# lattice/quda

Hardware: AMD Instinct MI355X
Metric: wilson_clover_cg_gflops (higher is better)
Workload: dtype double-half; 1 GPU; model=wilson_clover_eo_pc_cg, lattice_per_gpu=32x32x32x64, global_batch=1, seq_len=2097152, parallelism=dd_t1, gauge_recon_sloppy=12

## Files before the change

### csrc/bindings.cpp

```cpp
#include <torch/extension.h>
#include <c10/hip/HIPStream.h>
#include <hip/hip_runtime.h>

#include "launchers.h"

namespace {

int prec_of(const at::Tensor &t) {
  switch (t.scalar_type()) {
    case at::kDouble: return 0;
    case at::kFloat: return 1;
    case at::kHalf: return 2;
    case at::kFloat8_e4m3fn: return 3;
    default: TORCH_CHECK(false, "unsupported dtype");
  }
}

void *ptr_or_null(const at::Tensor &t) {
  return t.numel() ? t.data_ptr() : nullptr;
}

BlasField field_of(const at::Tensor &data, const at::Tensor &norm, long Vcb) {
  return BlasField{ptr_or_null(data), ptr_or_null(norm), Vcb};
}
// ... 263 lines not shown
}

static at::Tensor blas_op(int64_t op, double a, double b, at::Tensor x,
                          at::Tensor x_n, at::Tensor y, at::Tensor y_n,
                          int64_t Vcb, int64_t sites, double c2 = 0.0,
                          double d2 = 0.0, int64_t ncomp = 24,
                          bool deterministic = false,
                          c10::optional<at::Tensor> z = c10::nullopt,
                          c10::optional<at::Tensor> z_n = c10::nullopt,
                          c10::optional<at::Tensor> w = c10::nullopt,
                          c10::optional<at::Tensor> w_n = c10::nullopt) {
  TORCH_CHECK(op != BLAS_TRIPLE_CG_DEV,
              "blas_op: BLAS_TRIPLE_CG_DEV takes a device accumulator — call "
              "triple_cg_dev");
  BlasCall c{};
  c.op = (int)op;
  c.prec = prec_of(x);
  c.a = a;
  c.b = b;
  c.c = c2;
  c.d = d2;
  c.ncomp = (int)ncomp;
  c.det = deterministic;
  c.x = field_of(x, x_n, Vcb);
  c.y = field_of(y, y_n, Vcb);
  if (z) c.z = field_of(*z, *z_n, Vcb);
  if (w) c.w = field_of(*w, *w_n, Vcb);
  c.sites = sites;
  at::Tensor result;
  bool reduction = (op == BLAS_AXPY_NORM2 || op == BLAS_XMY_NORM2 ||
                    op == BLAS_NORM2 || op == BLAS_REDOT || op == BLAS_CDOT ||
                    op == BLAS_TRIPLE_CG);
  if (reduction) {
    if (deterministic) {
      long g = (sites + 255) / 256;
      if (g > 2048) g = 2048;
      result = at::zeros({g, 2}, x.options().dtype(at::kDouble));
    } else {
      result = at::zeros({2}, x.options().dtype(at::kDouble));
    }
    c.result = result.data_ptr<double>();
  }
  launch_blas(c, stream());
  check_launch("blas_op");
  if (reduction && deterministic) result = result.sum(0);
  return result;
}

static void triple_cg_dev(double r2_old, at::Tensor acc, at::Tensor clear,
                          at::Tensor p, at::Tensor p_n, at::Tensor Ap,
                          at::Tensor Ap_n, at::Tensor x, at::Tensor x_n,
                          at::Tensor r, at::Tensor r_n, int64_t Vcb,
                          int64_t sites, int64_t ncomp, at::Tensor slots,
                          int64_t nslots, int64_t slot_stride) {
  auto ok = [&](const at::Tensor &t) {
    return t.scalar_type() == at::kDouble && t.is_contiguous() &&
           t.device() == p.device();
  };
  TORCH_CHECK(ok(acc) && acc.numel() >= 2,
              "triple_cg_dev: acc must hold 2 float64 on the fields' device");
  TORCH_CHECK(clear.numel() == 0 || ok(clear),
              "triple_cg_dev: clear must be empty or float64 on the device");
  if (clear.numel()) {
    auto lo = (const char *)clear.data_ptr(), hi = lo + clear.numel() * 8;
    auto a0 = (const char *)acc.data_ptr();
    TORCH_CHECK(a0 + 16 <= lo || a0 >= hi,
                "triple_cg_dev: clear must not overlap acc");
  }
  TORCH_CHECK(nslots == 0 ||
              (ok(slots) && nslots >= 1 && nslots <= 64 && slot_stride >= 1 &&
               slots.numel() >= (nslots - 1) * slot_stride + 1),
              "triple_cg_dev: slots must hold nslots <= 64 strided float64");
  BlasCall c{};
  c.op = BLAS_TRIPLE_CG_DEV;
  c.prec = prec_of(p);
  c.a = r2_old;
  c.ncomp = (int)ncomp;
  c.x = field_of(p, p_n, Vcb);
  c.y = field_of(Ap, Ap_n, Vcb);
  c.z = field_of(x, x_n, Vcb);
  c.w = field_of(r, r_n, Vcb);
  c.sites = sites;
  c.result = acc.data_ptr<double>();
  c.clear = clear.numel() ? clear.data_ptr<double>() : nullptr;
  c.clear_n = clear.numel();
  c.nslots = (int)nslots;
  c.slot_stride = (int)slot_stride;
  c.slots = nslots ? slots.data_ptr<double>() : nullptr;
  launch_blas(c, stream());
  check_launch("triple_cg_dev");
}

static void convert(at::Tensor dst, at::Tensor dst_n, at::Tensor src,
                    at::Tensor src_n, int64_t Vcb, int64_t sites,
                    int64_t ncomp = 24) {
  launch_convert(field_of(dst, dst_n, Vcb), prec_of(dst),
                 field_of(src, src_n, Vcb), prec_of(src), sites, (int)ncomp,
                 stream());
  check_launch("convert");
}

static void clover_apply(at::Tensor out, at::Tensor out_n, at::Tensor in,
                         at::Tensor in_n, at::Tensor clover, int64_t parity,
                         int64_t Vcb, int64_t v_stride, int64_t s_offset) {
  CloverApplyCall c{};
  c.out = field_of_off(out, out_n, v_stride ? v_stride : Vcb, s_offset);
  c.in = field_of_off(in, in_n, v_stride ? v_stride : Vcb, s_offset);
  c.clover = clover.data_ptr();
  c.parity = (int)parity;
  c.Vcb = Vcb;
  c.sites = Vcb;
  c.prec = prec_of(out);
  launch_clover_apply(c, stream());
  check_launch("clover_apply");
}

static void twist_apply(at::Tensor out, at::Tensor out_n, at::Tensor in,
                        at::Tensor in_n, double b_re, double b_im,
                        int64_t Vcb, int64_t sites, int64_t tau3_vcb = 0,
                        bool acc = false) {
  TwistApplyCall c{};
  c.out = field_of(out, out_n, Vcb);
  c.in = field_of(in, in_n, Vcb);
  c.b_re = b_re;
  c.b_im = b_im;
  c.sites = sites;
  c.tau3_vcb = tau3_vcb;
  c.acc = acc;
  c.prec = prec_of(out);
  launch_twist_apply(c, stream());
  check_launch("twist_apply");
}

static void dwf5(at::Tensor out, at::Tensor out_n, at::Tensor in,
                 at::Tensor in_n, at::Tensor x, at::Tensor x_n,
                 int64_t Vcb4, int64_t Ls, bool xpay, bool dagger, double a,
                 double alpha, double beta, double mf, int64_t kind) {
  Dwf5Call c{};
  long stride = Vcb4 * Ls;
  c.out = field_of(out, out_n, stride);
  c.in = field_of(in, in_n, stride);
  c.x = field_of(x, x_n, stride);
  c.Vcb4 = Vcb4;
// ... 526 lines not shown
        py::arg("s_offsets") = std::vector<int64_t>{});
  m.def("flow_zmat_dir", &flow_zmat_dir, "wilson-flow Z = eps TA[S U^d]");
  m.def("flow_expmul_dir", &flow_expmul_dir, "U' = exp(Zc) U");
  m.def("stout_smear_dir", &stout_smear_dir,
        "native stout smear of one direction (exp via scale-and-square)");
  m.def("heatbath_sweep_dir", &heatbath_sweep_dir,
        "SU(2)-subgroup heatbath/overrelax update of one (parity, mu)");
  m.def("coarse_dslash_mfma", &coarse_dslash_mfma,
        "coarse-grid 9-matrix dslash on f32 MFMA tiles");
  m.def("dslash_staggered", &dslash_staggered, "naive staggered dslash");
  m.def("set_dslash_block", &set_dslash_block, "autotuner: dslash workgroup size");
  m.def("set_dslash_waves", &set_dslash_waves,
        "occupancy experiment: 0 default, 3 = 64-thread/3-wave variant "
        "(half/single/quarter; double keeps its default kernel)");
  m.def("set_dslash_lds", &set_dslash_lds,
        "LDS-tiled dslash policy: 1 = stage the in-spinor halo tile in LDS "
        "(half/quarter, local, tile-divisible dims)");
  m.def("get_dslash_block", &get_dslash_block, "current dslash workgroup size");
  m.def("get_dslash_lds", &get_dslash_lds, "current LDS-tiled dslash policy");
  m.def("get_dslash_waves", &get_dslash_waves, "current occupancy variant");
  m.def("ipc_get_handle", &ipc_get_handle, "hipIpcGetMemHandle of a tensor");
  m.def("ipc_open_handle", &ipc_open_handle, "open a peer IPC handle");
  m.def("ipc_close_handle", &ipc_close_handle, "close a peer IPC mapping");
  m.def("pack_face_ptr", &pack_face_ptr,
        "pack a halo face into a raw (IPC peer) pointer");
  m.def("dwf5", &dwf5, "DWF/Moebius 5th-dim ops (Ds apply / M5 inverse)");
  m.def("dwf_fused", &dwf_fused,
        "fused domain-wall kernel: out = [x +] a * W_chi (Dhat in), all Ls "
        "slices in one launch",
        py::arg("out"), py::arg("out_n"), py::arg("in"), py::arg("in_n"),
        py::arg("gauge"), py::arg("x"), py::arg("x_n"), py::arg("W"),
        py::arg("dims"), py::arg("parity_offset"), py::arg("Vcb"),
        py::arg("Ls"), py::arg("parity"), py::arg("dagger"), py::arg("xpay"),
        py::arg("a"), py::arg("recon"));
  m.def("set_dwf_fused_ns", &set_dwf_fused_ns,
        "fused domain-wall kernel: sites per workgroup for single/half "
        "(16 or 32)");
  m.attr("DWF_FUSED_LS_MAX") = (int)QA_DWF_FUSED_LS_MAX;
  m.def("zdwf5", &zdwf5, "zMobius per-slice-complex 5th-dim ops");
  m.def("eofa5", &eofa5, "EOFA rank-1 extended M5 ops");
  m.def("blas_op", &blas_op, "fused blas/reduction",
        py::arg("op"), py::arg("a"), py::arg("b"), py::arg("x"),
        py::arg("x_n"), py::arg("y"), py::arg("y_n"), py::arg("Vcb"),
        py::arg("sites"), py::arg("c2") = 0.0, py::arg("d2") = 0.0,
        py::arg("ncomp") = 24, py::arg("deterministic") = false,
        py::arg("z") = py::none(), py::arg("z_n") = py::none(),
        py::arg("w") = py::none(), py::arg("w_n") = py::none());
  m.def("triple_cg_dev", &triple_cg_dev,
        "fused CG update with alpha = r2_old / acc[0] formed on the device",
        py::arg("r2_old"), py::arg("acc"), py::arg("clear"), py::arg("p"),
        py::arg("p_n"), py::arg("Ap"), py::arg("Ap_n"), py::arg("x"),
        py::arg("x_n"), py::arg("r"), py::arg("r_n"), py::arg("Vcb"),
        py::arg("sites"), py::arg("ncomp"),
        py::arg("slots"), py::arg("nslots"), py::arg("slot_stride"));
  m.def("convert", &convert, "precision conversion copy", py::arg("dst"),
        py::arg("dst_n"), py::arg("src"), py::arg("src_n"), py::arg("Vcb"),
        py::arg("sites"), py::arg("ncomp") = 24);
  m.def("clover_apply", &clover_apply, "clover term apply",
        py::arg("out"), py::arg("out_n"), py::arg("in"), py::arg("in_n"),
        py::arg("clover"), py::arg("parity"), py::arg("Vcb"),
        py::arg("v_stride") = 0, py::arg("s_offset") = 0);
  m.def("twist_apply", &twist_apply, "twisted-mass T(b) apply",
        py::arg("out"), py::arg("out_n"), py::arg("in"), py::arg("in_n"),
        py::arg("b_re"), py::arg("b_im"), py::arg("Vcb"), py::arg("sites"),
        py::arg("tau3_vcb") = 0, py::arg("acc") = false);
  m.attr("BLAS_AXPY") = (int)BLAS_AXPY;
  m.attr("BLAS_AXPY_NORM2") = (int)BLAS_AXPY_NORM2;
  m.attr("BLAS_XPAY") = (int)BLAS_XPAY;
  m.attr("BLAS_AXPBY") = (int)BLAS_AXPBY;
  m.attr("BLAS_CAXPY") = (int)BLAS_CAXPY;
  m.attr("BLAS_XMY_NORM2") = (int)BLAS_XMY_NORM2;
  m.attr("BLAS_SCAL") = (int)BLAS_SCAL;
  m.attr("BLAS_NORM2") = (int)BLAS_NORM2;
  m.attr("BLAS_TRIPLE_CG") = (int)BLAS_TRIPLE_CG;
  m.attr("BLAS_TRIPLE_CG_DEV") = (int)BLAS_TRIPLE_CG_DEV;
  m.attr("BLAS_REDOT") = (int)BLAS_REDOT;
  m.attr("BLAS_CDOT") = (int)BLAS_CDOT;
  m.attr("BLAS_CAXPBY") = (int)BLAS_CAXPBY;
}
```

### csrc/blas.hip

```cpp
#include "common.h"
#include "reduce.h"

#define GRID_STRIDE(g, n)                                                     \
  for (long g = (long)blockIdx.x * blockDim.x + threadIdx.x; g < (n);         \
       g += (long)gridDim.x * blockDim.x)

template <typename A, bool NORM2>
__global__ __launch_bounds__(256) void k_axpy(
    typename A::R a, A x, A y, long sites, double *result, bool det) {
  using R = typename A::R;
  double acc = 0.0;
  GRID_STRIDE(g, sites) {
    cplx<R> xv[A::NCPLX], yv[A::NCPLX];
    x.load_v(xv, g);
    y.load_v(yv, g);
#pragma unroll
    for (int k = 0; k < A::NCPLX; ++k) {
      yv[k] = yv[k] + a * xv[k];
      if constexpr (NORM2)
        acc += (double)yv[k].re * yv[k].re + (double)yv[k].im * yv[k].im;
    }
    y.store_v(yv, g);
  }
  if constexpr (NORM2) block_atomic_add(acc, result, det, 2, 0);
// ... 114 lines not shown
  block_atomic_add(acc, result, det, 2, 0);
  if constexpr (KIND == 2) block_atomic_add(acc2, result, det, 2, 1);
}

template <typename AD, typename AS>
__global__ __launch_bounds__(256) void k_convert(AD dst, AS src, long sites) {
  using RS = typename AS::R;
  using RD = typename AD::R;
  static_assert(AD::NCPLX == AS::NCPLX);
  GRID_STRIDE(g, sites) {
    cplx<RS> v[AS::NCPLX];
    src.load_v(v, g);
    cplx<RD> o[AD::NCPLX];
#pragma unroll
    for (int k = 0; k < AS::NCPLX; ++k) o[k] = {(RD)v[k].re, (RD)v[k].im};
    dst.store_v(o, g);
  }
}

#include "launchers.h"

namespace {
constexpr int BLK = 256;
int grid_for(long sites) {
  long g = (sites + BLK - 1) / BLK;
  return (int)(g < 2048 ? g : 2048);
}
}

template <typename A>
__global__ __launch_bounds__(256) void k_triple_cg(
    typename A::R a, A p, A ap, A x, A r, long sites, double *result,
    bool det) {
  using R = typename A::R;
  double acc = 0.0;
  GRID_STRIDE(g, sites) {
    cplx<R> pv[A::NCPLX], av[A::NCPLX], xv[A::NCPLX], rv[A::NCPLX];
    p.load_v(pv, g);
    ap.load_v(av, g);
    x.load_v(xv, g);
    r.load_v(rv, g);
#pragma unroll
    for (int k = 0; k < A::NCPLX; ++k) {
      xv[k] = xv[k] + a * pv[k];
      rv[k] = rv[k] - a * av[k];
      acc += (double)rv[k].re * rv[k].re + (double)rv[k].im * rv[k].im;
    }
    x.store_v(xv, g);
    r.store_v(rv, g);
  }
  block_atomic_add(acc, result, det, 2, 0);
}

template <typename A>
__global__ __launch_bounds__(256) void k_triple_cg_dev(
    double r2_old, double *acc_out, double *clear, long clear_n,
    const double *slots, int nslots, int slot_stride, A p, A ap, A x, A r,
    long sites) {
  using R = typename A::R;
  if (clear && blockIdx.x == 0 && threadIdx.x < 64)
    for (long k = threadIdx.x; k < clear_n; k += 64) clear[k] = 0.0;
  double pAp;
  if (nslots > 0) {
    int lane = threadIdx.x & 63;
    double v = lane < nslots ? slots[(long)lane * slot_stride] : 0.0;
    v = wave_reduce(v);
    pAp = __shfl(v, 0, 64);
    if (blockIdx.x == 0 && threadIdx.x == 0) acc_out[0] = pAp;
  } else {
    pAp = acc_out[0];
  }
  if (pAp <= 0.0) return;
  const R a = (R)(r2_old / pAp);
  double acc = 0.0;
  GRID_STRIDE(g, sites) {
    cplx<R> pv[A::NCPLX], av[A::NCPLX], xv[A::NCPLX], rv[A::NCPLX];
    p.load_v(pv, g);
    ap.load_v(av, g);
    x.load_v(xv, g);
    r.load_v(rv, g);
#pragma unroll
    for (int k = 0; k < A::NCPLX; ++k) {
      xv[k] = xv[k] + a * pv[k];
      rv[k] = rv[k] - a * av[k];
      acc += (double)rv[k].re * rv[k].re + (double)rv[k].im * rv[k].im;
    }
    x.store_v(xv, g);
    r.store_v(rv, g);
  }
  block_atomic_add(acc, acc_out, false, 1, 1);
}

template <typename A>
static void blas_dispatch(const BlasCall &c, hipStream_t st) {
  using S = typename A::S;
  A x{(S *)c.x.data, (float *)c.x.norm, c.x.Vcb};
  A y{(S *)c.y.data, (float *)c.y.norm, c.y.Vcb};
  long n = c.sites;
  int gr = grid_for(n);
  using R = typename A::R;
  switch (c.op) {
    case BLAS_AXPY:
      hipLaunchKernelGGL((k_axpy<A, false>), dim3(gr), dim3(BLK), 0, st,
                         (R)c.a, x, y, n, nullptr, false);
      break;
    case BLAS_AXPY_NORM2:
      hipLaunchKernelGGL((k_axpy<A, true>), dim3(gr), dim3(BLK), 0, st,
                         (R)c.a, x, y, n, c.result, c.det);
      break;
    case BLAS_TRIPLE_CG: {
      A z{(S *)c.z.data, (float *)c.z.norm, c.z.Vcb};
      A w{(S *)c.w.data, (float *)c.w.norm, c.w.Vcb};
      hipLaunchKernelGGL((k_triple_cg<A>), dim3(gr), dim3(BLK), 0, st,
                         (R)c.a, x, y, z, w, n, c.result, c.det);
      break;
    }
    case BLAS_TRIPLE_CG_DEV: {
      A z{(S *)c.z.data, (float *)c.z.norm, c.z.Vcb};
      A w{(S *)c.w.data, (float *)c.w.norm, c.w.Vcb};
      hipLaunchKernelGGL((k_triple_cg_dev<A>), dim3(gr), dim3(BLK), 0, st,
                         c.a, c.result, c.clear, c.clear_n, c.slots, c.nslots,
                         c.slot_stride, x, y, z, w, n);
      break;
    }
    case BLAS_XPAY:
      hipLaunchKernelGGL((k_xpay<A>), dim3(gr), dim3(BLK), 0, st, x, (R)c.a, y, n);
      break;
    case BLAS_AXPBY:
      hipLaunchKernelGGL((k_axpby<A>), dim3(gr), dim3(BLK), 0, st, (R)c.a, x,
                         (R)c.b, y, n);
      break;
    case BLAS_CAXPY:
      hipLaunchKernelGGL((k_caxpy<A>), dim3(gr), dim3(BLK), 0, st, (R)c.a,
                         (R)c.b, x, y, n);
      break;
    case BLAS_CAXPBY:
      hipLaunchKernelGGL((k_caxpby<A>), dim3(gr), dim3(BLK), 0, st, (R)c.a,
                         (R)c.b, x, (R)c.c, (R)c.d, y, n);
      break;
    case BLAS_XMY_NORM2:
      hipLaunchKernelGGL((k_xmy_norm2<A>), dim3(gr), dim3(BLK), 0, st, x, y, n,
                         c.result, c.det);
      break;
    case BLAS_SCAL:
      hipLaunchKernelGGL((k_scal<A>), dim3(gr), dim3(BLK), 0, st, (R)c.a, x, n);
      break;
    case BLAS_NORM2:
      hipLaunchKernelGGL((k_reduce<A, 0>), dim3(gr), dim3(BLK), 0, st, x, y, n,
                         c.result, c.det);
      break;
    case BLAS_REDOT:
      hipLaunchKernelGGL((k_reduce<A, 1>), dim3(gr), dim3(BLK), 0, st, x, y, n,
                         c.result, c.det);
      break;
    case BLAS_CDOT:
      hipLaunchKernelGGL((k_reduce<A, 2>), dim3(gr), dim3(BLK), 0, st, x, y, n,
                         c.result, c.det);
      break;
  }
}

void launch_blas(const BlasCall &c, hipStream_t st) {
  if (c.ncomp == 6) {
    switch (c.prec) {
      case 0: blas_dispatch<StagAcc<PrecDouble>>(c, st); break;
      case 1: blas_dispatch<StagAcc<PrecSingle>>(c, st); break;
      case 2: blas_dispatch<StagAcc<PrecHalf>>(c, st); break;
      case 3: blas_dispatch<StagAcc<PrecQuarter>>(c, st); break;
    }
  } else {
    switch (c.prec) {
      case 0: blas_dispatch<SpinorAcc<PrecDouble>>(c, st); break;
      case 1: blas_dispatch<SpinorAcc<PrecSingle>>(c, st); break;
      case 2: blas_dispatch<SpinorAcc<PrecHalf>>(c, st); break;
      case 3: blas_dispatch<SpinorAcc<PrecQuarter>>(c, st); break;
    }
  }
}

template <template <typename> class AT, typename PD, typename PS>
static void conv(const BlasField &d, const BlasField &s, long sites, hipStream_t st) {
  auto da = AT<PD>{(typename PD::Store *)d.data, (float *)d.norm, d.Vcb};
  auto sa = AT<PS>{(typename PS::Store *)s.data, (float *)s.norm, s.Vcb};
  hipLaunchKernelGGL((k_convert<AT<PD>, AT<PS>>), dim3(grid_for(sites)),
                     dim3(BLK), 0, st, da, sa, sites);
}

template <template <typename> class AT>
static void conv_dispatch(const BlasField &dst, int pdst, const BlasField &src,
                          int psrc, long sites, hipStream_t st) {
  switch (pdst * 4 + psrc) {
    case 0 * 4 + 1: conv<AT, PrecDouble, PrecSingle>(dst, src, sites, st); break;
    case 0 * 4 + 2: conv<AT, PrecDouble, PrecHalf>(dst, src, sites, st); break;
    case 1 * 4 + 0: conv<AT, PrecSingle, PrecDouble>(dst, src, sites, st); break;
    case 1 * 4 + 2: conv<AT, PrecSingle, PrecHalf>(dst, src, sites, st); break;
    case 2 * 4 + 0: conv<AT, PrecHalf, PrecDouble>(dst, src, sites, st); break;
    case 2 * 4 + 1: conv<AT, PrecHalf, PrecSingle>(dst, src, sites, st); break;
    case 0 * 4 + 0: conv<AT, PrecDouble, PrecDouble>(dst, src, sites, st); break;
    case 1 * 4 + 1: conv<AT, PrecSingle, PrecSingle>(dst, src, sites, st); break;
    case 2 * 4 + 2: conv<AT, PrecHalf, PrecHalf>(dst, src, sites, st); break;
    case 0 * 4 + 3: conv<AT, PrecDouble, PrecQuarter>(dst, src, sites, st); break;
    case 1 * 4 + 3: conv<AT, PrecSingle, PrecQuarter>(dst, src, sites, st); break;
    case 2 * 4 + 3: conv<AT, PrecHalf, PrecQuarter>(dst, src, sites, st); break;
    case 3 * 4 + 0: conv<AT, PrecQuarter, PrecDouble>(dst, src, sites, st); break;
    case 3 * 4 + 1: conv<AT, PrecQuarter, PrecSingle>(dst, src, sites, st); break;
    case 3 * 4 + 2: conv<AT, PrecQuarter, PrecHalf>(dst, src, sites, st); break;
    case 3 * 4 + 3: conv<AT, PrecQuarter, PrecQuarter>(dst, src, sites, st); break;
  }
}

template <typename P>
using WilsonAccT = SpinorAcc<P, 24>;

void launch_convert(const BlasField &dst, int pdst, const BlasField &src,
                    int psrc, long sites, int ncomp, hipStream_t st) {
  if (ncomp == 6)
    conv_dispatch<StagAcc>(dst, pdst, src, psrc, sites, st);
  else
    conv_dispatch<WilsonAccT>(dst, pdst, src, psrc, sites, st);
}
```

### csrc/launchers.h

```cpp
#pragma once
#include <hip/hip_runtime.h>

#include <cstdlib>

inline int &qa_dslash_block_ref() {
  static int blk = [] {
    const char *e = getenv("QUDA_AMD_DSLASH_BLOCK");
    int v = e ? atoi(e) : 64;
    return (v == 64 || v == 128 || v == 256) ? v : 64;
  }();
  return blk;
}
inline int qa_dslash_block() { return qa_dslash_block_ref(); }

inline int &qa_dslash_waves_ref() {
  static int w = [] {
    const char *e = getenv("QUDA_AMD_DSLASH_WAVES");
    int v = e ? atoi(e) : 0;
    return v == 3 ? 3 : 0;
  }();
  return w;
}
inline int qa_dslash_waves() { return qa_dslash_waves_ref(); }

inline int &qa_dslash_lds_ref() {
  static int v = []() {
    const char *e = std::getenv("QUDA_AMD_DSLASH_LDS");
    return e ? std::atoi(e) : 0;
  }();
  return v;
}
inline int qa_dslash_lds() { return qa_dslash_lds_ref(); }

struct BlasField {
  void *data;
  void *norm;
  long Vcb;
};

enum BlasOp {
  BLAS_AXPY = 0,
  BLAS_AXPY_NORM2,
  BLAS_XPAY,
  BLAS_AXPBY,
  BLAS_CAXPY,
  BLAS_XMY_NORM2,
  BLAS_SCAL,
  BLAS_NORM2,
  BLAS_REDOT,
  BLAS_CDOT,
  BLAS_CAXPBY,
  BLAS_TRIPLE_CG,
  BLAS_TRIPLE_CG_DEV,
};

struct BlasCall {
  int op;
  int prec;
  double a, b;
  double c, d;
  BlasField x, y;
  BlasField z, w;
  long sites;
  int ncomp;
  bool det;
  double *result;
  double *clear;
  long clear_n;
  const double *slots;
  int nslots, slot_stride;
};

void launch_blas(const BlasCall &c, hipStream_t st);
void launch_convert(const BlasField &dst, int pdst, const BlasField &src,
                    int psrc, long sites, int ncomp, hipStream_t st);

struct LatDesc {
  int Xdim[4];
  int parity_offset;
  long Vcb;
};

struct GhostDesc {
  const void *ghost[8];
  const float *ghost_nrm[8];
  long face_cb[4];
  int comm_mask;
};

struct DslashCall {
  BlasField out, in, x;
  const void *gauge;
  const void *clover;
  LatDesc lat;
  int parity;
  bool dagger;
  int mode;
  bool xpay;
  double a;
  double b_re, b_im;
  int recon;
  GhostDesc halo;
  int kt;
  BlasField out2, y;
  double *dot_result;
  int dot_slots, dot_stride;
};

inline bool qa_dslash_epilogue_ok(const DslashCall &c) {
  if (!c.out2.data && !c.y.data) return true;
  if (c.kt != 0 && c.kt != 1) return false;
  if (qa_dslash_waves() != 0) return false;
  if (c.y.data && (c.dot_slots < 1 || c.dot_stride < 1)) return false;
  if (c.out2.data && c.y.data) return false;
  if (c.out2.data) return c.mode == 1 && !c.dagger;
  if (c.y.data) return c.mode == 0 && c.dagger && c.xpay && c.dot_result;
  return true;
}

void launch_dslash_wilson_double(const DslashCall &c, hipStream_t st);
void launch_dslash_wilson_single(const DslashCall &c, hipStream_t st);
void launch_dslash_wilson_half(const DslashCall &c, hipStream_t st);
void launch_dslash_wilson_quarter(const DslashCall &c, hipStream_t st);

#define QA_MRHS_MAX 4
struct DslashMrhsCall {
// ... 224 lines not shown
```

### quda_amd/ops/blas.py

```python

from __future__ import annotations

import torch

from ..fields.spinor import SpinorField
from ..parallel.comms import allreduce_sum
from .dispatch import hip_ext, norm_or_empty, on_gpu


def _is_half(x: SpinorField) -> bool:
    return x.precision in ("half", "quarter")


def _pairs(t: torch.Tensor) -> torch.Tensor:
    return t.reshape(*t.shape[:-1], t.shape[-1] // 2, 2)


def _requant(x: SpinorField, vals: torch.Tensor):
    x.from_complex(vals.reshape(x.n_parity, x.volume_cb, *x.site_shape))


def _cvals(x: SpinorField) -> torch.Tensor:
    return x.to_complex(torch.complex128).reshape(x.n_parity, x.volume_cb,
                                                  x.ncomp // 2)
# ... 42 lines not shown
    if on_gpu(x, y):
        ext = hip_ext()
        r = _gpu_blas(ext.BLAS_REDOT, 0, 0, x, y)[0].item()
    elif _is_half(x) or _is_half(y):
        r = (_cvals(x).conj() * _cvals(y)).real.sum().item()
    else:
        r = (x.data.to(torch.float64) * y.data.to(torch.float64)).sum().item()
    return allreduce_sum(r)


def c_dot(x: SpinorField, y: SpinorField) -> complex:
    if on_gpu(x, y):
        ext = hip_ext()
        t = _gpu_blas(ext.BLAS_CDOT, 0, 0, x, y)
        re, im = t[0].item(), t[1].item()
        return complex(allreduce_sum(re), allreduce_sum(im))
    if _is_half(x) or _is_half(y):
        s = (_cvals(x).conj() * _cvals(y)).sum().item()
        return complex(allreduce_sum(s.real), allreduce_sum(s.imag))
    px, py = _pairs(x.data.to(torch.float64)), _pairs(y.data.to(torch.float64))
    re = (px * py).sum().item()
    im = (px[..., 0] * py[..., 1] - px[..., 1] * py[..., 0]).sum().item()
    return complex(allreduce_sum(re), allreduce_sum(im))


def axpy_norm2(a: float, x: SpinorField, y: SpinorField) -> float:
    if on_gpu(x, y):
        ext = hip_ext()
        r = _gpu_blas(ext.BLAS_AXPY_NORM2, a, 0, x, y)[0].item()
        return allreduce_sum(r)
    axpy(a, x, y)
    return norm2(y)


def triple_cg_update(a: float, p: SpinorField, Ap: SpinorField,
                     x: SpinorField, r: SpinorField) -> float:
    if on_gpu(p, Ap, x, r):
        ext = hip_ext()
        res = ext.blas_op(ext.BLAS_TRIPLE_CG, float(a), 0.0, p.data,
                          norm_or_empty(p), Ap.data, norm_or_empty(Ap),
                          p.volume_cb, p.n_parity * p.volume_cb,
                          ncomp=p.ncomp,
                          deterministic=deterministic_reductions(),
                          z=x.data, z_n=norm_or_empty(x),
                          w=r.data, w_n=norm_or_empty(r))
        return allreduce_sum(res[0].item())
    axpy(a, p, x)
    return axpy_norm2(-a, Ap, r)


def triple_cg_update_dev(r2_old: float, acc: torch.Tensor, clear,
                         p: SpinorField, Ap: SpinorField, x: SpinorField,
                         r: SpinorField, slots=None, nslots: int = 0,
                         slot_stride: int = 1) -> None:
    assert on_gpu(p, Ap, x, r), "triple_cg_update_dev: GPU fields only"
    ext = hip_ext()
    empty = torch.empty(0, dtype=torch.float64, device=acc.device)
    ext.triple_cg_dev(float(r2_old), acc, empty if clear is None else clear,
                      p.data, norm_or_empty(p), Ap.data, norm_or_empty(Ap),
                      x.data, norm_or_empty(x), r.data, norm_or_empty(r),
                      p.volume_cb, p.n_parity * p.volume_cb, p.ncomp,
                      empty if slots is None else slots, int(nslots),
                      int(slot_stride))


def xmy_norm2(x: SpinorField, y: SpinorField) -> float:
    if on_gpu(x, y):
        ext = hip_ext()
        r = _gpu_blas(ext.BLAS_XMY_NORM2, 0, 0, x, y)[0].item()
        return allreduce_sum(r)
    if _is_half(x) or _is_half(y):
        v = _cvals(x) - _cvals(y)
        _requant(y, v)
        return allreduce_sum((v.real ** 2 + v.imag ** 2).sum().item())
    y.data.copy_(x.data - y.data)
    return norm2(y)



def copy(dst: SpinorField, src: SpinorField) -> SpinorField:
    if dst is src:
        return dst
    if on_gpu(dst, src) and dst.precision != src.precision:
        ext = hip_ext()
        ext.convert(dst.data, norm_or_empty(dst), src.data, norm_or_empty(src),
                    dst.volume_cb, dst.n_parity * dst.volume_cb,
                    ncomp=dst.ncomp)
        return dst
    dst.copy_(src)
    return dst


def zero(x: SpinorField) -> SpinorField:
    return x.zero_()


def axpy(a: float, x: SpinorField, y: SpinorField) -> SpinorField:
    if on_gpu(x, y):
        ext = hip_ext()
        _gpu_blas(ext.BLAS_AXPY, a, 0, x, y)
    elif _is_half(x) or _is_half(y):
        _requant(y, _cvals(y) + a * _cvals(x))
    else:
        y.data.add_(x.data.to(y.data.dtype), alpha=float(a))
    return y


def xpay(x: SpinorField, a: float, y: SpinorField) -> SpinorField:
    if on_gpu(x, y):
        ext = hip_ext()
        _gpu_blas(ext.BLAS_XPAY, a, 0, x, y)
    elif _is_half(x) or _is_half(y):
        _requant(y, _cvals(x) + a * _cvals(y))
    else:
        y.data.mul_(float(a)).add_(x.data.to(y.data.dtype))
    return y
# ... 58 lines not shown
```

### quda_amd/solvers/cg.py

```python

from __future__ import annotations

from dataclasses import dataclass, field
from math import sqrt
from typing import Callable, Optional

from ..fields.spinor import SpinorField
from ..ops import blas


@dataclass
class SolverStats:
    iters: int = 0
    resid: float = 0.0
    true_resid: float = 0.0
    reliable_updates: int = 0
    converged: bool = False
    hq_resid: float = 0.0
    flops: float = 0.0
    seconds: float = 0.0


def hq_residual(x: SpinorField, r: SpinorField) -> float:
    import torch
    xv = x.to_complex()
    rv = r.to_complex()
    dims = tuple(range(2, xv.dim()))
    x2 = xv.abs().square().sum(dim=dims).clamp_min(1e-300)
    r2 = rv.abs().square().sum(dim=dims)
    from ..parallel import comms
    num = comms.allreduce_sum(float((r2 / x2).sum()))
    den = comms.allreduce_sum(float(x2.numel()))
    return sqrt(num / den)


_SLOTS = 32
_STRIDE = 16


def cg_solve(op, x: SpinorField, b: SpinorField, *,
             op_sloppy=None, sloppy: Optional[str] = None,
             tol: float = 1e-8, maxiter: int = 1000,
             delta: float = 0.1, hq_tol: float = 0.0) -> SolverStats:
    stats = SolverStats()
    prec_hi = x.precision
    sloppy = sloppy or prec_hi
    op_sloppy = op_sloppy or op
    geo, dev, npar, nsp, nls = x.geo, x.device, x.n_parity, x.nspin, x.ls

    def hi():
        return SpinorField(geo, prec_hi, dev, npar, nspin=nsp, ls=nls)

    def lo():
        return SpinorField(geo, sloppy, dev, npar, nspin=nsp, ls=nls)

    b2 = blas.norm2(b)
    if b2 == 0.0:
        x.zero_()
        stats.converged = True
        return stats
    stop = tol * tol * b2

    r = hi()
    tmp_hi = hi()
    x2 = blas.norm2(x)
    if x2 > 0.0:
        op.MdagM(r, x, tmp_hi)
        r2 = blas.xmy_norm2(b, r)
    else:
        blas.copy(r, b)
        r2 = b2

    mixed = (sloppy != prec_hi) or (op_sloppy is not op)
    r_s = lo()
    p = lo()
    Ap = lo()
    x_s = lo()
    tmp_s = lo()
    blas.copy(r_s, r)
    blas.copy(p, r_s)
    x_s.zero_()

    maxr = sqrt(r2)
    k = 0
    x_s_dirty = False
    from ..ops.dispatch import on_gpu
    from ..parallel import comms
    fused_dot = (hasattr(op_sloppy, "MdagM_dot") and on_gpu(p, Ap)
                 and not comms.is_distributed()
                 and not blas.deterministic_reductions())
    if fused_dot:
        import torch
        n_acc = _STRIDE * (1 + _SLOTS)
        acc = torch.zeros(2 * n_acc, dtype=torch.float64,
                          device=p.data.device)
        accs = (acc[:n_acc], acc[n_acc:])
        heads = tuple(a[:2] for a in accs)
        slots = tuple(a[_STRIDE:] for a in accs)
    while r2 > stop and k < maxiter:
        if fused_dot:
            cur = k & 1
            op_sloppy.MdagM_dot(Ap, p, tmp_s, slots[cur], _SLOTS, _STRIDE)
            blas.triple_cg_update_dev(r2, heads[cur], accs[1 - cur], p, Ap,
                                      x_s, r_s, slots[cur], _SLOTS, _STRIDE)
            pAp, r2_new = heads[cur].tolist()
            if pAp <= 0.0:
                break
            x_s_dirty = True
            r2_old = r2
            r2 = r2_new
        else:
            op_sloppy.MdagM(Ap, p, tmp_s)
            pAp = blas.re_dot(p, Ap)
            if pAp <= 0.0:
                break
            alpha = r2 / pAp
            x_s_dirty = True
            r2_old = r2
            r2 = blas.triple_cg_update(alpha, p, Ap, x_s, r_s)
        k += 1
        rnorm = sqrt(r2)
        maxr = max(maxr, rnorm)

        need_reliable = mixed and (rnorm < delta * maxr)
        if need_reliable or r2 <= stop:
            blas.copy(tmp_hi, x_s)
            blas.axpy(1.0, tmp_hi, x)
            op.MdagM(r, x, tmp_hi)
            r2 = blas.xmy_norm2(b, r)
            x_s.zero_()
            x_s_dirty = False
            blas.copy(r_s, r)
            beta = r2 / r2_old
            blas.xpay(r_s, beta, p)
            maxr = sqrt(r2)
            stats.reliable_updates += 1
            if r2 <= stop:
                break
        else:
            beta = r2 / r2_old
            blas.xpay(r_s, beta, p)

    if x_s_dirty:
        blas.copy(tmp_hi, x_s)
        blas.axpy(1.0, tmp_hi, x)
        op.MdagM(r, x, tmp_hi)
        r2 = blas.xmy_norm2(b, r)

    stats.iters = k
    stats.resid = sqrt(r2 / b2)
    stats.true_resid = stats.resid
    stats.converged = r2 <= stop
    if hq_tol > 0.0 and stats.converged:
        stats.hq_resid = hq_residual(x, r)
        if stats.hq_resid > hq_tol:
            extra = 0
            while stats.hq_resid > hq_tol and k + extra < maxiter:
                st2 = cg_solve(op, x, b, op_sloppy=op_sloppy,
                               sloppy=sloppy, tol=stats.resid * 0.1,
                               maxiter=maxiter - k - extra, delta=delta)
                extra += st2.iters
                op.MdagM(r, x, tmp_hi)
                blas.xmy_norm2(b, r)
                stats.hq_resid = hq_residual(x, r)
                if st2.iters == 0:
                    break
            stats.iters = k + extra
            stats.converged = stats.hq_resid <= hq_tol
    return stats
```

Baseline: 13670 GFLOPS.

## Move CG tail update and reliable-update decision onto the device

Splits the sloppy CG iteration. The triple update now skips the x update and is followed by a device tail kernel. That kernel forms alpha, beta and the reliable-update decision on the device, then does x += alpha p and either p = r + beta p or x only. Scalars are copied back asynchronously on a side stream into pinned memory, so the host no longer needs a separate xpay launch after its readback. Reliable updates use fused fold and residual-restart kernels in place of copy/axpy/zero chains. This adds host/device decision consistency checks and a side-stream synchronisation per iteration.

```diff
diff --git a/csrc/bindings.cpp b/csrc/bindings.cpp
--- a/csrc/bindings.cpp
+++ b/csrc/bindings.cpp
@@ -339,7 +339,8 @@
                           at::Tensor Ap_n, at::Tensor x, at::Tensor x_n,
                           at::Tensor r, at::Tensor r_n, int64_t Vcb,
                           int64_t sites, int64_t ncomp, at::Tensor slots,
-                          int64_t nslots, int64_t slot_stride) {
+                          int64_t nslots, int64_t slot_stride,
+                          bool update_x = true) {
   auto ok = [&](const at::Tensor &t) {
     return t.scalar_type() == at::kDouble && t.is_contiguous() &&
            t.device() == p.device();
@@ -374,8 +375,112 @@
   c.nslots = (int)nslots;
   c.slot_stride = (int)slot_stride;
   c.slots = nslots ? slots.data_ptr<double>() : nullptr;
+  c.skip_x = !update_x;
   launch_blas(c, stream());
   check_launch("triple_cg_dev");
+}
+
+static void check_field(const char *what, const at::Tensor &t,
+                        const at::Tensor &t_n, const at::Tensor &ref,
+                        bool same_dtype, int64_t sites, int64_t ncomp) {
+  TORCH_CHECK(t.is_contiguous() && t.device() == ref.device() &&
+                  (!same_dtype || t.scalar_type() == ref.scalar_type()) &&
+                  t.numel() >= sites * ncomp,
+              what, ": field does not match the call");
+  bool normed = t.scalar_type() == at::kHalf ||
+                t.scalar_type() == at::kFloat8_e4m3fn;
+  TORCH_CHECK(!normed || (t_n.scalar_type() == at::kFloat &&
+                          t_n.is_contiguous() && t_n.device() == ref.device() &&
+                          t_n.numel() >= sites),
+              what, ": half/quarter field without its per-site norms");
+}
+
+static void cg_tail_dev(double r2_old, double maxr, double delta, double stop,
+                        bool mixed, double tag, at::Tensor acc,
+                        at::Tensor status, at::Tensor p, at::Tensor p_n,
+                        at::Tensor x, at::Tensor x_n, at::Tensor r,
+                        at::Tensor r_n, int64_t Vcb, int64_t sites,
+                        int64_t ncomp) {
+  auto ok = [&](const at::Tensor &t, int64_t n) {
+    return t.scalar_type() == at::kDouble && t.is_contiguous() &&
+           t.device() == p.device() && t.numel() >= n;
+  };
+  TORCH_CHECK(ok(acc, 2) && ok(status, 1),
+              "cg_tail_dev: acc (2) and status (1) must be float64 on the "
+              "fields' device");
+  TORCH_CHECK(ncomp == 24 || ncomp == 6, "cg_tail_dev: ncomp must be 24 or 6");
+  TORCH_CHECK(sites >= 0 && Vcb > 0 && sites % Vcb == 0 && sites / Vcb <= 2,
+              "cg_tail_dev: sites must be one or two parities of Vcb");
+  check_field("cg_tail_dev p", p, p_n, p, true, sites, ncomp);
+  check_field("cg_tail_dev x", x, x_n, p, true, sites, ncomp);
+  check_field("cg_tail_dev r", r, r_n, p, true, sites, ncomp);
+  CgTailCall c{};
+  c.r2_old = r2_old;
+  c.maxr = maxr;
+  c.delta = delta;
+  c.stop = stop;
+  c.mixed = mixed;
+  c.tag = tag;
+  c.acc = acc.data_ptr<double>();
+  c.status = status.data_ptr<double>();
+  c.p = field_of(p, p_n, Vcb);
+  c.x = field_of(x, x_n, Vcb);
+  c.r = field_of(r, r_n, Vcb);
+  c.sites = sites;
+  c.ncomp = (int)ncomp;
+  c.prec = prec_of(p);
+  launch_cg_tail(c, stream());
+  check_launch("cg_tail_dev");
+}
+
+static void reliable_check(const char *what, const at::Tensor &hi,
+                           const at::Tensor &hi_n, const at::Tensor &lo,
+                           const at::Tensor &lo_n, int64_t Vcb, int64_t sites,
+                           int64_t ncomp) {
+  TORCH_CHECK(qa_reliable_prec_ok(prec_of(hi)), what,
+              ": the precise field must be double or single");
+  TORCH_CHECK(ncomp == 24 || ncomp == 6, what, ": ncomp must be 24 or 6");
+  TORCH_CHECK(sites >= 0 && Vcb > 0 && sites % Vcb == 0 && sites / Vcb <= 2,
+              what, ": sites must be one or two parities of Vcb");
+  check_field(what, hi, hi_n, hi, true, sites, ncomp);
+  check_field(what, lo, lo_n, hi, false, sites, ncomp);
+}
+
+static void fold_sloppy(at::Tensor x, at::Tensor x_n, at::Tensor xs,
+                        at::Tensor xs_n, int64_t Vcb, int64_t sites,
+                        int64_t ncomp) {
+  reliable_check("fold_sloppy", x, x_n, xs, xs_n, Vcb, sites, ncomp);
+  ReliableCall c{};
+  c.kind = 0;
+  c.hi = field_of(x, x_n, Vcb);
+  c.lo = field_of(xs, xs_n, Vcb);
+  c.prec_hi = prec_of(x);
+  c.prec_lo = prec_of(xs);
+  c.sites = sites;
+  c.ncomp = (int)ncomp;
+  launch_reliable(c, stream());
+  check_launch("fold_sloppy");
+}
+
+static at::Tensor resid_restart(at::Tensor b, at::Tensor b_n, at::Tensor r,
+                                at::Tensor r_n, at::Tensor rs, at::Tensor rs_n,
+                                int64_t Vcb, int64_t sites, int64_t ncomp) {
+  reliable_check("resid_restart", r, r_n, rs, rs_n, Vcb, sites, ncomp);
+  check_field("resid_restart b", b, b_n, r, true, sites, ncomp);
+  at::Tensor result = at::zeros({2}, r.options().dtype(at::kDouble));
+  ReliableCall c{};
+  c.kind = 1;
+  c.hi = field_of(r, r_n, Vcb);
+  c.b = field_of(b, b_n, Vcb);
+  c.lo = field_of(rs, rs_n, Vcb);
+  c.prec_hi = prec_of(r);
+  c.prec_lo = prec_of(rs);
+  c.sites = sites;
+  c.ncomp = (int)ncomp;
+  c.result = result.data_ptr<double>();
+  launch_reliable(c, stream());
+  check_launch("resid_restart");
+  return result;
 }
 
 static void convert(at::Tensor dst, at::Tensor dst_n, at::Tensor src,
@@ -1008,7 +1113,24 @@
         py::arg("p_n"), py::arg("Ap"), py::arg("Ap_n"), py::arg("x"),
         py::arg("x_n"), py::arg("r"), py::arg("r_n"), py::arg("Vcb"),
         py::arg("sites"), py::arg("ncomp"),
-        py::arg("slots"), py::arg("nslots"), py::arg("slot_stride"));
+        py::arg("slots"), py::arg("nslots"), py::arg("slot_stride"),
+        py::arg("update_x") = true);
+  m.def("cg_tail_dev", &cg_tail_dev,
+        "second half of a sloppy CG iteration: x += alpha p and, unless a "
+        "reliable update is due, p = r + beta p, scalars formed on the device",
+        py::arg("r2_old"), py::arg("maxr"), py::arg("delta"), py::arg("stop"),
+        py::arg("mixed"), py::arg("tag"), py::arg("acc"), py::arg("status"),
+        py::arg("p"), py::arg("p_n"), py::arg("x"), py::arg("x_n"),
+        py::arg("r"), py::arg("r_n"), py::arg("Vcb"), py::arg("sites"),
+        py::arg("ncomp"));
+  m.def("fold_sloppy", &fold_sloppy, "reliable update: x += x_s; x_s = 0",
+        py::arg("x"), py::arg("x_n"), py::arg("xs"), py::arg("xs_n"),
+        py::arg("Vcb"), py::arg("sites"), py::arg("ncomp"));
+  m.def("resid_restart", &resid_restart,
+        "reliable update: r = b - r; r_s = r; returns ||r||^2",
+        py::arg("b"), py::arg("b_n"), py::arg("r"), py::arg("r_n"),
+        py::arg("rs"), py::arg("rs_n"), py::arg("Vcb"), py::arg("sites"),
+        py::arg("ncomp"));
   m.def("convert", &convert, "precision conversion copy", py::arg("dst"),
         py::arg("dst_n"), py::arg("src"), py::arg("src_n"), py::arg("Vcb"),
         py::arg("sites"), py::arg("ncomp") = 24);
diff --git a/csrc/blas.hip b/csrc/blas.hip
--- a/csrc/blas.hip
+++ b/csrc/blas.hip
@@ -190,7 +190,7 @@
   block_atomic_add(acc, result, det, 2, 0);
 }
 
-template <typename A>
+template <typename A, bool UPDATE_X = true>
 __global__ __launch_bounds__(256) void k_triple_cg_dev(
     double r2_old, double *acc_out, double *clear, long clear_n,
     const double *slots, int nslots, int slot_stride, A p, A ap, A x, A r,
@@ -213,20 +213,111 @@
   double acc = 0.0;
   GRID_STRIDE(g, sites) {
     cplx<R> pv[A::NCPLX], av[A::NCPLX], xv[A::NCPLX], rv[A::NCPLX];
-    p.load_v(pv, g);
+    if constexpr (UPDATE_X) p.load_v(pv, g);
     ap.load_v(av, g);
-    x.load_v(xv, g);
+    if constexpr (UPDATE_X) x.load_v(xv, g);
     r.load_v(rv, g);
 #pragma unroll
     for (int k = 0; k < A::NCPLX; ++k) {
-      xv[k] = xv[k] + a * pv[k];
+      if constexpr (UPDATE_X) xv[k] = xv[k] + a * pv[k];
       rv[k] = rv[k] - a * av[k];
       acc += (double)rv[k].re * rv[k].re + (double)rv[k].im * rv[k].im;
     }
+    if constexpr (UPDATE_X) x.store_v(xv, g);
+    r.store_v(rv, g);
+  }
+  block_atomic_add(acc, acc_out, false, 1, 1);
+}
+
+template <typename A>
+__global__ __launch_bounds__(256) void k_cg_tail_dev(
+    double r2_old, double maxr, double delta, double stop, bool mixed,
+    double tag, const double *acc, double *status, A p, A x, A r,
+    long sites) {
+  using R = typename A::R;
+  const double pAp = acc[0];
+  const double r2 = acc[1];
+  const bool first = blockIdx.x == 0 && threadIdx.x == 0;
+  if (pAp <= 0.0) {
+    if (first) *status = -tag;
+    return;
+  }
+  const R a = (R)(r2_old / pAp);
+  const double rnorm = __dsqrt_rn(r2);
+  const double maxr_new = rnorm > maxr ? rnorm : maxr;
+  const bool need = (mixed && rnorm < delta * maxr_new) || r2 <= stop;
+  if (first) *status = 2.0 * tag + (need ? 1.0 : 0.0);
+  if (need) {
+    GRID_STRIDE(g, sites) {
+      cplx<R> pv[A::NCPLX], xv[A::NCPLX];
+      p.load_v(pv, g);
+      x.load_v(xv, g);
+#pragma unroll
+      for (int k = 0; k < A::NCPLX; ++k)
+        xv[k] = {fma(a, pv[k].re, xv[k].re), fma(a, pv[k].im, xv[k].im)};
+      x.store_v(xv, g);
+    }
+    return;
+  }
+  const R b = (R)(r2 / r2_old);
+  GRID_STRIDE(g, sites) {
+    cplx<R> pv[A::NCPLX], xv[A::NCPLX], rv[A::NCPLX];
+    p.load_v(pv, g);
+    x.load_v(xv, g);
+    r.load_v(rv, g);
+#pragma unroll
+    for (int k = 0; k < A::NCPLX; ++k) {
+      xv[k] = {fma(a, pv[k].re, xv[k].re), fma(a, pv[k].im, xv[k].im)};
+      pv[k] = {fma(b, pv[k].re, rv[k].re), fma(b, pv[k].im, rv[k].im)};
+    }
     x.store_v(xv, g);
+    p.store_v(pv, g);
+  }
+}
+
+template <typename AH, typename AL>
+__global__ __launch_bounds__(256) void k_fold_sloppy(AH x, AL xs, long sites) {
+  using RH = typename AH::R;
+  using RL = typename AL::R;
+  static_assert(AH::NCPLX == AL::NCPLX);
+  GRID_STRIDE(g, sites) {
+    cplx<RL> sv[AL::NCPLX];
+    cplx<RH> xv[AH::NCPLX];
+    xs.load_v(sv, g);
+    x.load_v(xv, g);
+#pragma unroll
+    for (int k = 0; k < AH::NCPLX; ++k) {
+#pragma clang fp contract(off)
+      xv[k] = {xv[k].re + (RH)sv[k].re, xv[k].im + (RH)sv[k].im};
+      sv[k] = {(RL)0, (RL)0};
+    }
+    x.store_v(xv, g);
+    xs.store_v(sv, g);
+  }
+}
+
+template <typename AH, typename AL>
+__global__ __launch_bounds__(256) void k_resid_restart(
+    AH b, AH r, AL rs, long sites, double *result) {
+  using RH = typename AH::R;
+  using RL = typename AL::R;
+  static_assert(AH::NCPLX == AL::NCPLX);
+  double acc = 0.0;
+  GRID_STRIDE(g, sites) {
+    cplx<RH> bv[AH::NCPLX], rv[AH::NCPLX];
+    cplx<RL> sv[AL::NCPLX];
+    b.load_v(bv, g);
+    r.load_v(rv, g);
+#pragma unroll
+    for (int k = 0; k < AH::NCPLX; ++k) {
+      rv[k] = bv[k] - rv[k];
+      acc += (double)rv[k].re * rv[k].re + (double)rv[k].im * rv[k].im;
+      sv[k] = {(RL)rv[k].re, (RL)rv[k].im};
+    }
     r.store_v(rv, g);
-  }
-  block_atomic_add(acc, acc_out, false, 1, 1);
+    rs.store_v(sv, g);
+  }
+  block_atomic_add(acc, result, false, 2, 0);
 }
 
 template <typename A>
@@ -256,9 +347,14 @@
     case BLAS_TRIPLE_CG_DEV: {
       A z{(S *)c.z.data, (float *)c.z.norm, c.z.Vcb};
       A w{(S *)c.w.data, (float *)c.w.norm, c.w.Vcb};
-      hipLaunchKernelGGL((k_triple_cg_dev<A>), dim3(gr), dim3(BLK), 0, st,
-                         c.a, c.result, c.clear, c.clear_n, c.slots, c.nslots,
-                         c.slot_stride, x, y, z, w, n);
+      if (!c.skip_x)
+        hipLaunchKernelGGL((k_triple_cg_dev<A, true>), dim3(gr), dim3(BLK), 0,
+                           st, c.a, c.result, c.clear, c.clear_n, c.slots,
+                           c.nslots, c.slot_stride, x, y, z, w, n);
+      else
+        hipLaunchKernelGGL((k_triple_cg_dev<A, false>), dim3(gr), dim3(BLK), 0,
+                           st, c.a, c.result, c.clear, c.clear_n, c.slots,
+                           c.nslots, c.slot_stride, x, y, z, w, n);
       break;
     }
     case BLAS_XPAY:
@@ -314,6 +410,75 @@
       case 3: blas_dispatch<SpinorAcc<PrecQuarter>>(c, st); break;
     }
   }
+}
+
+template <typename A>
+static void cg_tail_dispatch(const CgTailCall &c, hipStream_t st) {
+  using S = typename A::S;
+  A p{(S *)c.p.data, (float *)c.p.norm, c.p.Vcb};
+  A x{(S *)c.x.data, (float *)c.x.norm, c.x.Vcb};
+  A r{(S *)c.r.data, (float *)c.r.norm, c.r.Vcb};
+  hipLaunchKernelGGL((k_cg_tail_dev<A>), dim3(grid_for(c.sites)), dim3(BLK), 0,
+                     st, c.r2_old, c.maxr, c.delta, c.stop, c.mixed, c.tag,
+                     c.acc, c.status, p, x, r, c.sites);
+}
+
+void launch_cg_tail(const CgTailCall &c, hipStream_t st) {
+  if (c.ncomp == 6) {
+    switch (c.prec) {
+      case 0: cg_tail_dispatch<StagAcc<PrecDouble>>(c, st); break;
+      case 1: cg_tail_dispatch<StagAcc<PrecSingle>>(c, st); break;
+      case 2: cg_tail_dispatch<StagAcc<PrecHalf>>(c, st); break;
+      case 3: cg_tail_dispatch<StagAcc<PrecQuarter>>(c, st); break;
+    }
+  } else {
+    switch (c.prec) {
+      case 0: cg_tail_dispatch<SpinorAcc<PrecDouble>>(c, st); break;
+      case 1: cg_tail_dispatch<SpinorAcc<PrecSingle>>(c, st); break;
+      case 2: cg_tail_dispatch<SpinorAcc<PrecHalf>>(c, st); break;
+      case 3: cg_tail_dispatch<SpinorAcc<PrecQuarter>>(c, st); break;
+    }
+  }
+}
+
+template <template <typename> class AT, typename PH, typename PL>
+static void reliable_launch(const ReliableCall &c, hipStream_t st) {
+  auto hi = [](const BlasField &f) {
+    return AT<PH>{(typename PH::Store *)f.data, (float *)f.norm, f.Vcb};
+  };
+  auto lo = AT<PL>{(typename PL::Store *)c.lo.data, (float *)c.lo.norm,
+                   c.lo.Vcb};
+  int gr = grid_for(c.sites);
+  if (c.kind == 0)
+    hipLaunchKernelGGL((k_fold_sloppy<AT<PH>, AT<PL>>), dim3(gr), dim3(BLK), 0,
+                       st, hi(c.hi), lo, c.sites);
+  else
+    hipLaunchKernelGGL((k_resid_restart<AT<PH>, AT<PL>>), dim3(gr), dim3(BLK),
+                       0, st, hi(c.b), hi(c.hi), lo, c.sites, c.result);
+}
+
+template <template <typename> class AT>
+static void reliable_dispatch(const ReliableCall &c, hipStream_t st) {
+  switch (c.prec_hi * 4 + c.prec_lo) {
+    case 0 * 4 + 0: reliable_launch<AT, PrecDouble, PrecDouble>(c, st); break;
+    case 0 * 4 + 1: reliable_launch<AT, PrecDouble, PrecSingle>(c, st); break;
+    case 0 * 4 + 2: reliable_launch<AT, PrecDouble, PrecHalf>(c, st); break;
+    case 0 * 4 + 3: reliable_launch<AT, PrecDouble, PrecQuarter>(c, st); break;
+    case 1 * 4 + 0: reliable_launch<AT, PrecSingle, PrecDouble>(c, st); break;
+    case 1 * 4 + 1: reliable_launch<AT, PrecSingle, PrecSingle>(c, st); break;
+    case 1 * 4 + 2: reliable_launch<AT, PrecSingle, PrecHalf>(c, st); break;
+    case 1 * 4 + 3: reliable_launch<AT, PrecSingle, PrecQuarter>(c, st); break;
+  }
+}
+
+template <typename P>
+using WilsonAccR = SpinorAcc<P, 24>;
+
+void launch_reliable(const ReliableCall &c, hipStream_t st) {
+  if (c.ncomp == 6)
+    reliable_dispatch<StagAcc>(c, st);
+  else
+    reliable_dispatch<WilsonAccR>(c, st);
 }
 
 template <template <typename> class AT, typename PD, typename PS>
diff --git a/csrc/launchers.h b/csrc/launchers.h
--- a/csrc/launchers.h
+++ b/csrc/launchers.h
@@ -69,9 +69,34 @@
   long clear_n;
   const double *slots;
   int nslots, slot_stride;
+  bool skip_x;
 };
 
 void launch_blas(const BlasCall &c, hipStream_t st);
+
+struct CgTailCall {
+  double r2_old, maxr, delta, stop;
+  bool mixed;
+  double tag;
+  const double *acc;
+  double *status;
+  BlasField p, x, r;
+  long sites;
+  int ncomp;
+  int prec;
+};
+void launch_cg_tail(const CgTailCall &c, hipStream_t st);
+
+struct ReliableCall {
+  int kind;
+  BlasField hi, b, lo;
+  int prec_hi, prec_lo;
+  long sites;
+  int ncomp;
+  double *result;
+};
+inline bool qa_reliable_prec_ok(int prec_hi) { return prec_hi == 0 || prec_hi == 1; }
+void launch_reliable(const ReliableCall &c, hipStream_t st);
 void launch_convert(const BlasField &dst, int pdst, const BlasField &src,
                     int psrc, long sites, int ncomp, hipStream_t st);
 
diff --git a/quda_amd/ops/blas.py b/quda_amd/ops/blas.py
--- a/quda_amd/ops/blas.py
+++ b/quda_amd/ops/blas.py
@@ -118,7 +118,7 @@
 def triple_cg_update_dev(r2_old: float, acc: torch.Tensor, clear,
                          p: SpinorField, Ap: SpinorField, x: SpinorField,
                          r: SpinorField, slots=None, nslots: int = 0,
-                         slot_stride: int = 1) -> None:
+                         slot_stride: int = 1, update_x: bool = True) -> None:
     assert on_gpu(p, Ap, x, r), "triple_cg_update_dev: GPU fields only"
     ext = hip_ext()
     empty = torch.empty(0, dtype=torch.float64, device=acc.device)
@@ -127,7 +127,42 @@
                       x.data, norm_or_empty(x), r.data, norm_or_empty(r),
                       p.volume_cb, p.n_parity * p.volume_cb, p.ncomp,
                       empty if slots is None else slots, int(nslots),
-                      int(slot_stride))
+                      int(slot_stride), bool(update_x))
+
+
+def cg_tail_dev(r2_old: float, maxr: float, delta: float, stop: float,
+                mixed: bool, tag: int, acc: torch.Tensor,
+                status: torch.Tensor, p: SpinorField, x: SpinorField,
+                r: SpinorField) -> None:
+    assert on_gpu(p, x, r), "cg_tail_dev: GPU fields only"
+    ext = hip_ext()
+    ext.cg_tail_dev(float(r2_old), float(maxr), float(delta), float(stop),
+                    bool(mixed), float(tag), acc, status,
+                    p.data, norm_or_empty(p), x.data, norm_or_empty(x),
+                    r.data, norm_or_empty(r), p.volume_cb,
+                    p.n_parity * p.volume_cb, p.ncomp)
+
+
+def reliable_kernels_ok(x: SpinorField, x_s: SpinorField) -> bool:
+    return (on_gpu(x, x_s) and x.precision in ("double", "single")
+            and not deterministic_reductions())
+
+
+def fold_sloppy(x: SpinorField, x_s: SpinorField) -> None:
+    assert reliable_kernels_ok(x, x_s), "fold_sloppy: no kernel for this pair"
+    hip_ext().fold_sloppy(x.data, norm_or_empty(x), x_s.data,
+                          norm_or_empty(x_s), x.volume_cb,
+                          x.n_parity * x.volume_cb, x.ncomp)
+
+
+def resid_restart(b: SpinorField, r: SpinorField, r_s: SpinorField) -> float:
+    assert reliable_kernels_ok(r, r_s) and on_gpu(b), \
+        "resid_restart: no kernel for this pair"
+    res = hip_ext().resid_restart(b.data, norm_or_empty(b), r.data,
+                                  norm_or_empty(r), r_s.data,
+                                  norm_or_empty(r_s), r.volume_cb,
+                                  r.n_parity * r.volume_cb, r.ncomp)
+    return allreduce_sum(res[0].item())
 
 
 def xmy_norm2(x: SpinorField, y: SpinorField) -> float:
diff --git a/quda_amd/solvers/cg.py b/quda_amd/solvers/cg.py
--- a/quda_amd/solvers/cg.py
+++ b/quda_amd/solvers/cg.py
@@ -38,6 +38,19 @@
 _STRIDE = 16
 
 
+def tail_decision(r2: float, maxr: float, delta: float, stop: float,
+                  mixed: bool):
+    rnorm = sqrt(r2)
+    maxr = max(maxr, rnorm)
+    need = (mixed and rnorm < delta * maxr) or r2 <= stop
+    return rnorm, maxr, need
+
+
+def device_tail_enabled() -> bool:
+    import os
+    return os.environ.get("QUDA_AMD_CG_DEVICE_TAIL", "1") != "0"
+
+
 def cg_solve(op, x: SpinorField, b: SpinorField, *,
              op_sloppy=None, sloppy: Optional[str] = None,
              tol: float = 1e-8, maxiter: int = 1000,
@@ -89,16 +102,61 @@
     fused_dot = (hasattr(op_sloppy, "MdagM_dot") and on_gpu(p, Ap)
                  and not comms.is_distributed()
                  and not blas.deterministic_reductions())
+    device_tail = device_tail_enabled()
+    fused_ru = device_tail and blas.reliable_kernels_ok(x, x_s)
+    use_tail = fused_dot and device_tail
     if fused_dot:
         import torch
         n_acc = _STRIDE * (1 + _SLOTS)
-        acc = torch.zeros(2 * n_acc, dtype=torch.float64,
+        n_blk = _STRIDE + n_acc
+        acc = torch.zeros(2 * n_blk, dtype=torch.float64,
                           device=p.data.device)
-        accs = (acc[:n_acc], acc[n_acc:])
+        accs = tuple(acc[i * n_blk + _STRIDE:(i + 1) * n_blk] for i in (0, 1))
         heads = tuple(a[:2] for a in accs)
         slots = tuple(a[_STRIDE:] for a in accs)
+    if use_tail:
+        reads = tuple(acc[i * n_blk + _STRIDE - 1:i * n_blk + _STRIDE + 2]
+                      for i in (0, 1))
+        report = tuple(rd[:1] for rd in reads)
+        fetched = torch.empty(3, dtype=torch.float64).pin_memory()
+        side = torch.cuda.Stream(device=acc.device)
+        done = torch.cuda.Event()
+        expect = None
+        last_report = None
+
+    def check_report(seen):
+        if seen != expect:
+            raise RuntimeError(
+                f"cg_solve: host and device disagree on the end of sloppy "
+                f"iteration {k}: device reported {seen!r}, host expected "
+                f"{expect!r} (2 * iteration + reliable update due, or "
+                f"-iteration on breakdown)")
+
     while r2 > stop and k < maxiter:
-        if fused_dot:
+        if use_tail:
+            cur = k & 1
+            op_sloppy.MdagM_dot(Ap, p, tmp_s, slots[cur], _SLOTS, _STRIDE)
+            blas.triple_cg_update_dev(r2, heads[cur], accs[1 - cur], p, Ap,
+                                      x_s, r_s, slots[cur], _SLOTS, _STRIDE,
+                                      update_x=False)
+            done.record(torch.cuda.current_stream(acc.device))
+            blas.cg_tail_dev(r2, maxr, delta, stop, mixed, k + 1, heads[cur],
+                             report[1 - cur], p, x_s, r_s)
+            with torch.cuda.stream(side):
+                side.wait_event(done)
+                fetched.copy_(reads[cur], non_blocking=True)
+            side.synchronize()
+            seen, pAp, r2_new = fetched.tolist()
+            if expect is not None:
+                check_report(seen)
+            last_report = report[1 - cur]
+            if pAp <= 0.0:
+                expect = -float(k + 1)
+                break
+            x_s_dirty = True
+            r2_old = r2
+            r2 = r2_new
+        elif fused_dot:
             cur = k & 1
             op_sloppy.MdagM_dot(Ap, p, tmp_s, slots[cur], _SLOTS, _STRIDE)
             blas.triple_cg_update_dev(r2, heads[cur], accs[1 - cur], p, Ap,
@@ -119,31 +177,42 @@
             r2_old = r2
             r2 = blas.triple_cg_update(alpha, p, Ap, x_s, r_s)
         k += 1
-        rnorm = sqrt(r2)
-        maxr = max(maxr, rnorm)
-
-        need_reliable = mixed and (rnorm < delta * maxr)
-        if need_reliable or r2 <= stop:
-            blas.copy(tmp_hi, x_s)
-            blas.axpy(1.0, tmp_hi, x)
-            op.MdagM(r, x, tmp_hi)
-            r2 = blas.xmy_norm2(b, r)
-            x_s.zero_()
+        rnorm, maxr, need = tail_decision(r2, maxr, delta, stop, mixed)
+        if use_tail:
+            expect = float(2 * k + need)
+
+        if need:
+            if fused_ru:
+                blas.fold_sloppy(x, x_s)
+                op.MdagM(r, x, tmp_hi)
+                r2 = blas.resid_restart(b, r, r_s)
+            else:
+                blas.copy(tmp_hi, x_s)
+                blas.axpy(1.0, tmp_hi, x)
+                op.MdagM(r, x, tmp_hi)
+                r2 = blas.xmy_norm2(b, r)
+                x_s.zero_()
+                blas.copy(r_s, r)
             x_s_dirty = False
-            blas.copy(r_s, r)
             beta = r2 / r2_old
             blas.xpay(r_s, beta, p)
             maxr = sqrt(r2)
             stats.reliable_updates += 1
             if r2 <= stop:
                 break
-        else:
+        elif not use_tail:
             beta = r2 / r2_old
             blas.xpay(r_s, beta, p)
 
+    if use_tail and expect is not None:
+        check_report(last_report.item())
+
     if x_s_dirty:
-        blas.copy(tmp_hi, x_s)
-        blas.axpy(1.0, tmp_hi, x)
+        if fused_ru:
+            blas.fold_sloppy(x, x_s)
+        else:
+            blas.copy(tmp_hi, x_s)
+            blas.axpy(1.0, tmp_hi, x)
         op.MdagM(r, x, tmp_hi)
         r2 = blas.xmy_norm2(b, r)
 
```

After: 13840 GFLOPS (median of 2 runs). No clear change (+1.2%).
